# menyifang/MIMO

Measured on NVIDIA H100. Metric: frames/sec @ 512x512x24f, 20 DDIM steps, higher is better.
Workload: dtype fp16

## Files before the change

mimo_b200/csrc/gemm_wgmma.cu:

```cuda
#include <cuda_runtime.h>

#include <cudaTypedefs.h>

#include "../../include/mimo_b200.h"
#include "host_util.h"
#include "ptx.cuh"
#include "wgmma.cuh"

namespace mimo {

constexpr int BM = 128;
constexpr int BK = 64;
constexpr int kGemmThreads = 320;
constexpr int kChunk = 8192;

struct EpiArgs {
  const void* bias;
  const void* rowvec;
  long long rows_per_group;
  long long ld_rowvec;
  float scale;
  int act;
  float* partial;
};

struct ConvGeom {
  int conv;
  int H, W, NI;
  int TW, TH, TN;
  int tiles_w, tiles_h;
  int ctot;
  int c0;
  int kb0, kb1;
  int a_bytes;
  int chunk_bytes;
  int splits;
  int kb_split;
  int ntaps;
  signed char tdx[9], tdy[9];
};

template <int BN, bool kRes>
struct GemmCfg {
  static constexpr int kStageBytes = BM * BK * 2 + BN * BK * 2;
  static constexpr int kNChunk = BN / 32;
  static constexpr int kOutBytes = 2 * kChunk;
  static constexpr int kResSlots = kRes ? 2 : 0;
  static constexpr int kResBytes = kResSlots * kChunk;
  static constexpr int kBarBytes = 512;
  static constexpr int kFixed = kBarBytes + 2048  + kOutBytes + kResBytes;
  static constexpr int kMaxStages = (BN >= 256) ? 4 : (BN >= 160 ? 5 : (BN >= 128 ? 6 : 8));
  static constexpr int kFit = (227 * 1024 - kFixed) / kStageBytes;
  static constexpr int kStages = kFit < kMaxStages ? kFit : kMaxStages;
  static constexpr int kSmemBytes = kStages * kStageBytes + kFixed;
  static_assert(kStages >= 3, "pipeline too shallow");
};

template <int BN, bool kBf16, bool kRes>
__global__ void __launch_bounds__(kGemmThreads, 1)
gemm_wgmma_kernel(const __grid_constant__ CUtensorMap tmA0, const __grid_constant__ CUtensorMap tmA1,
                  const __grid_constant__ CUtensorMap tmB, const __grid_constant__ CUtensorMap tmOut,
                  const __grid_constant__ CUtensorMap tmRes, int M, int N, int num_m_tiles, int num_n_tiles,
                  int num_k_blocks, ConvGeom g, EpiArgs ep) {
  using Cfg = GemmCfg<BN, kRes>;
  using C = Cvt<kBf16>;
  using T = typename C::T;
  constexpr int NCHUNK = Cfg::kNChunk;
  extern __shared__ __align__(1024) uint8_t smem[];
  uint8_t* sOut = smem + Cfg::kStages * Cfg::kStageBytes;
  uint8_t* sRes = sOut + Cfg::kOutBytes;
  uint64_t* bars = reinterpret_cast<uint64_t*>(sRes + Cfg::kResBytes);
  uint64_t* full_bar = bars;
  uint64_t* empty_bar = bars + 8;
  uint64_t* res_full = bars + 16;
  uint64_t* res_empty = bars + 18;
  float* sbias = reinterpret_cast<float*>(reinterpret_cast<uint8_t*>(bars) + Cfg::kBarBytes);

  pdl_launch_dependents();
  const int warp = __shfl_sync(0xffffffffu, threadIdx.x >> 5, 0);
  const int lane = threadIdx.x & 31;
  const int num_tiles = num_m_tiles * num_n_tiles * g.splits;
  auto decode = [&](int tile, int& m_tile, int& n_tile, int& split, int& kb_begin, int& kb_cnt) {
    const int mn = tile / g.splits;
    split = tile - mn * g.splits;
    m_tile = mn / num_n_tiles;
    n_tile = mn - m_tile * num_n_tiles;
    kb_begin = split * g.kb_split;
    kb_cnt = num_k_blocks - kb_begin;
    if (kb_cnt > g.kb_split) kb_cnt = g.kb_split;
  };

  if (warp == 8 && lane == 0) {
    tma_prefetch_desc(&tmA0);
    tma_prefetch_desc(&tmA1);
    tma_prefetch_desc(&tmB);
    tma_prefetch_desc(&tmOut);
    if (kRes) tma_prefetch_desc(&tmRes);
  }
  if (warp == 9 && lane == 0) {
    for (int s = 0; s < Cfg::kStages; ++s) {
      mbar_init(&full_bar[s], 1);
      mbar_init(&empty_bar[s], 8);
    }
    for (int s = 0; s < Cfg::kResSlots; ++s) {
      mbar_init(&res_full[s], 1);
      mbar_init(&res_empty[s], 8);
    }
    fence_mbar_init();
  }
  __syncthreads();
  pdl_wait();

  auto tile_origin = [&](int m_tile, int& x0, int& y0, int& n0) {
    if (g.conv) {
      x0 = (m_tile % g.tiles_w) * g.TW;
      y0 = ((m_tile / g.tiles_w) % g.tiles_h) * g.TH;
      n0 = (m_tile / (g.tiles_w * g.tiles_h)) * g.TN;
    } else {
      x0 = y0 = n0 = 0;
    }
  };

  if (warp == 8) {
    uint32_t stage = 0, phase = 0;
    const int kb_per_tap = g.kb0 + g.kb1;
    for (int tile = blockIdx.x; tile < num_tiles; tile += gridDim.x) {
      int m_tile, n_tile, split, kb_begin, kb_cnt;
      decode(tile, m_tile, n_tile, split, kb_begin, kb_cnt);
      int x0, y0, n0;
      tile_origin(m_tile, x0, y0, n0);
      int tap = kb_per_tap > 0 ? kb_begin / kb_per_tap : 0;
      int rem = kb_begin - tap * kb_per_tap;
      int dx = g.tdx[tap], dy = g.tdy[tap], tap_k = tap * g.ctot;
      for (int kbl = 0, kb = kb_begin; kbl < kb_cnt; ++kbl, ++kb) {
        mbar_wait(&empty_bar[stage], phase ^ 1u);
        uint8_t* sa = smem + stage * Cfg::kStageBytes;
        uint8_t* sb = sa + BM * BK * 2;
        if (elect_one()) {
          if (!g.conv) {
            mbar_expect_tx(&full_bar[stage], BM * BK * 2 + BN * BK * 2);
            if (kb < g.kb0) {
              tma_load_2d(sa, &tmA0, &full_bar[stage], kb * BK, m_tile * BM);
              tma_load_2d(sb, &tmB, &full_bar[stage], kb * BK, n_tile * BN);
            } else {
              tma_load_2d(sa, &tmA1, &full_bar[stage], (kb - g.kb0) * BK, m_tile * BM);
              tma_load_2d(sb, &tmB, &full_bar[stage], g.c0 + (kb - g.kb0) * BK, n_tile * BN);
            }
          } else {
            mbar_expect_tx(&full_bar[stage], g.a_bytes + BN * BK * 2);
            int kcoord;
            if (rem < g.kb0) {
              tma_load_4d(sa, &tmA0, &full_bar[stage], rem * BK, x0 + dx, y0 + dy, n0);
              kcoord = tap_k + rem * BK;
            } else {
              tma_load_4d(sa, &tmA1, &full_bar[stage], (rem - g.kb0) * BK, x0 + dx, y0 + dy, n0);
              kcoord = tap_k + g.c0 + (rem - g.kb0) * BK;
            }
            tma_load_2d(sb, &tmB, &full_bar[stage], kcoord, n_tile * BN);
          }
        }
        __syncwarp();
        if (++rem == kb_per_tap) {
          rem = 0;
          tap_k += g.ctot;
          if (++tap == g.ntaps) tap = 0;
          dx = g.tdx[tap];
          dy = g.tdy[tap];
        }
        if (++stage == Cfg::kStages) {
          stage = 0;
          phase ^= 1u;
        }
      }
    }
  } else if (warp == 9) {
    if constexpr (kRes) {
      uint32_t k = 0;
      for (int tile = blockIdx.x; tile < num_tiles; tile += gridDim.x) {
        const int m_tile = tile / num_n_tiles;
        const int n_tile = tile % num_n_tiles;
        int x0, y0, n0;
        tile_origin(m_tile, x0, y0, n0);
        for (int c = 0; c < NCHUNK; ++c, ++k) {
          const uint32_t slot = k % Cfg::kResSlots;
          mbar_wait(&res_empty[slot], ((k / Cfg::kResSlots) & 1u) ^ 1u);
          if (elect_one()) {
            mbar_expect_tx(&res_full[slot], g.chunk_bytes);
            const int col = n_tile * BN + c * 32;
            if (g.conv)
              tma_load_4d(sRes + slot * kChunk, &tmRes, &res_full[slot], col, x0, y0, n0);
            else
              tma_load_2d(sRes + slot * kChunk, &tmRes, &res_full[slot], col, m_tile * BM);
          }
          __syncwarp();
        }
      }
    }
  } else if (warp < 8) {
    const int wg = warp >> 2;
    const int ct = threadIdx.x;
    const int rbase = wg * 64 + (warp & 3) * 16 + (lane >> 2);
    const int q2 = (lane & 3) * 2;
    const bool issuer = ct == 0;
    const int sw[2] = {(rbase >> 1) & 3, ((rbase + 8) >> 1) & 3};
    const bool do_silu = ep.act == MIMO_ACT_SILU;
    const uint32_t rpg = static_cast<uint32_t>(ep.rows_per_group);
    float acc[BN / 2];
    uint32_t stage = 0, phase = 0, lt = 0, oc = 0, rc = 0;

    for (int tile = blockIdx.x; tile < num_tiles; tile += gridDim.x, ++lt) {
      int m_tile, n_tile, split, kb_begin, kb_cnt;
      decode(tile, m_tile, n_tile, split, kb_begin, kb_cnt);
      int x0, y0, n0;
      tile_origin(m_tile, x0, y0, n0);
      auto tile_groups = [&](int mt, uint32_t& gf, uint32_t& gl) {
        if (!g.conv) {
          const uint32_t m0 = static_cast<uint32_t>(mt) * BM;
          uint32_t m1 = m0 + BM - 1;
          if (m1 > static_cast<uint32_t>(M) - 1) m1 = static_cast<uint32_t>(M) - 1;
          gf = m0 / rpg;
          gl = m1 / rpg;
        } else {
          int tx, ty, tn;
          tile_origin(mt, tx, ty, tn);
          int n1 = tn + g.TN - 1;
          if (n1 > g.NI - 1) n1 = g.NI - 1;
          const uint32_t hw = static_cast<uint32_t>(g.H) * g.W;
          gf = (static_cast<uint32_t>(tn) * hw) / rpg;
          gl = (static_cast<uint32_t>(n1 + 1) * hw - 1) / rpg;
        }
      };
      const int ce = ct;
      auto load_consts = [&](int t) -> float {
        float v = 0.f;
        const int mt = (t / g.splits) / num_n_tiles, nt = (t / g.splits) % num_n_tiles;
        const int col = nt * BN + ce;
        if (ce < BN && col < N) {
          if (ep.bias) v = C::to_f(static_cast<const T*>(ep.bias)[col]);
          if (ep.rowvec) {
            uint32_t gf, gl;
            tile_groups(mt, gf, gl);
            if (gf == gl) v += C::to_f(static_cast<const T*>(ep.rowvec)[static_cast<long long>(gf) * ep.ld_rowvec + col]);
          }
        }
        return ep.act == MIMO_ACT_GEGLU ? v : v * ep.scale;
      };
      float* sb = sbias + (lt & 1u) * 256;
      if (ct < BN) sb[ct] = load_consts(tile);

      uint32_t prev_stage = 0;
      for (int kb = 0; kb < kb_cnt; ++kb) {
        mbar_wait(&full_bar[stage], phase);
        const uint32_t sa = smem_u32(smem + stage * Cfg::kStageBytes);
        const uint64_t da = make_smem_desc_sw128(sa + wg * (64 * 128), 16, 1024);
        const uint64_t db = make_smem_desc_sw128(sa + BM * BK * 2, 16, 1024);
        wgmma_fence();
#pragma unroll
        for (int k = 0; k < BK / 16; ++k) {
          Wgmma<BN, kBf16>::ss(acc, da + 2 * k, db + 2 * k, (kb | k) != 0 ? 1u : 0u);
        }
        wgmma_commit();
        if (kb > 0) {
          wgmma_wait<1>();
          if (lane == 0) mbar_arrive(&empty_bar[prev_stage]);
        }
        prev_stage = stage;
        if (++stage == Cfg::kStages) {
          stage = 0;
          phase ^= 1u;
        }
      }
      wgmma_wait<0>();
      reg_fence(acc);
      if (lane == 0) mbar_arrive(&empty_bar[prev_stage]);

      long long row[2];
      bool row_ok[2];
#pragma unroll
      for (int h = 0; h < 2; ++h) {
        const int r = rbase + 8 * h;
        if (!g.conv) {
          row[h] = static_cast<long long>(m_tile) * BM + r;
          row_ok[h] = row[h] < M;
        } else {
          const int x = r % g.TW, y = (r / g.TW) % g.TH, n = r / (g.TW * g.TH);
          row_ok[h] = (n < g.TN) && (x0 + x < g.W) && (y0 + y < g.H) && (n0 + n < g.NI);
          row[h] = (static_cast<long long>(n0 + n) * g.H + (y0 + y)) * g.W + (x0 + x);
        }
      }
      asm volatile("bar.sync 1, 256;" ::: "memory");

      if (ep.partial) {
#pragma unroll
        for (int h = 0; h < 2; ++h) {
          if (!row_ok[h]) continue;
          float* prow = ep.partial + (static_cast<long long>(split) * M + row[h]) * N;
#pragma unroll
          for (int j = 0; j < BN / 8; ++j) {
            const int col = n_tile * BN + 8 * j + q2;
            if (col < N) *reinterpret_cast<float2*>(prow + col) = make_float2(acc[4 * j + 2 * h], acc[4 * j + 2 * h + 1]);
          }
        }
        continue;
      }

      auto stage_and_store = [&](uint8_t* obuf, int col0) {
        fence_proxy_async_smem();
        if (issuer) tma_store_wait_read0();
        asm volatile("bar.sync 1, 256;" ::: "memory");
        if (issuer) {
          if (g.conv)
            tma_store_4d(&tmOut, obuf, col0, x0, y0, n0);
          else
            tma_store_2d(&tmOut, obuf, col0, m_tile * BM);
          tma_store_commit();
        }
      };

      if (ep.act != MIMO_ACT_GEGLU) {
        const float scale = ep.scale;
        bool rv_uniform = false;
        if (ep.rowvec) {
          uint32_t gf, gl;
          tile_groups(m_tile, gf, gl);
          rv_uniform = gf == gl;
        }
        const bool need_rv = ep.rowvec != nullptr && !rv_uniform;
        const int mode = (!kRes && !do_silu && !need_rv && ep.bias == nullptr && ep.rowvec == nullptr && scale == 1.0f)
                             ? 0 : (need_rv ? 2 : 1);
        const T* rv[2];
#pragma unroll
        for (int h = 0; h < 2; ++h)
          rv[h] = (need_rv && row_ok[h])
                      ? static_cast<const T*>(ep.rowvec) + static_cast<long long>(static_cast<uint32_t>(row[h]) / rpg) * ep.ld_rowvec
                      : nullptr;
#pragma unroll
        for (int c = 0; c < NCHUNK; ++c) {
          uint8_t* obuf = sOut + (oc & 1u) * kChunk;
          ++oc;
          const int col0 = n_tile * BN + c * 32;
          [[maybe_unused]] uint32_t rslot = 0;
          if constexpr (kRes) {
            const uint32_t k = rc++;
            rslot = k % Cfg::kResSlots;
            mbar_wait(&res_full[rslot], (k / Cfg::kResSlots) & 1u);
          }
#pragma unroll
          for (int jj = 0; jj < 4; ++jj) {
            const int j = 4 * c + jj;
            const float2 cst0 = *reinterpret_cast<const float2*>(sb + c * 32 + 8 * jj + q2);
#pragma unroll
            for (int h = 0; h < 2; ++h) {
              const int r = rbase + 8 * h;
              const int off = r * 64 + ((jj ^ sw[h]) << 4) + q2 * 2;
              float f0 = acc[4 * j + 2 * h], f1 = acc[4 * j + 2 * h + 1];
              if (mode != 0) {
                float c0 = cst0.x, c1 = cst0.y;
                if (mode == 2 && rv[h] && col0 + 8 * jj + q2 < N) {
                  const float2 t = C::unpack(__ldg(reinterpret_cast<const unsigned int*>(rv[h] + col0 + 8 * jj + q2)));
                  c0 = fmaf(t.x, scale, c0);
                  c1 = fmaf(t.y, scale, c1);
                }
                f0 = fmaf(f0, scale, c0);
                f1 = fmaf(f1, scale, c1);
              }
              if constexpr (kRes) {
                const float2 t = C::unpack(*reinterpret_cast<const uint32_t*>(sRes + rslot * kChunk + off));
                f0 = fmaf(t.x, scale, f0);
                f1 = fmaf(t.y, scale, f1);
              }
              if (do_silu) {
                f0 = silu_f(f0);
                f1 = silu_f(f1);
              }
              *reinterpret_cast<uint32_t*>(obuf + off) = C::pack(f0, f1);
            }
          }
          if constexpr (kRes) {
            __syncwarp();
            if (lane == 0) mbar_arrive(&res_empty[rslot]);
          }
          stage_and_store(obuf, col0);
        }
      } else {
        constexpr int HALF = BN / 2;
#pragma unroll
        for (int c = 0; c < HALF / 32; ++c) {
          uint8_t* obuf = sOut + (oc & 1u) * kChunk;
          ++oc;
#pragma unroll
          for (int jj = 0; jj < 4; ++jj) {
            const int j = 4 * c + jj, jg = j + HALF / 8;
            const float2 cv = *reinterpret_cast<const float2*>(sb + c * 32 + 8 * jj + q2);
            const float2 cg = *reinterpret_cast<const float2*>(sb + HALF + c * 32 + 8 * jj + q2);
#pragma unroll
            for (int h = 0; h < 2; ++h) {
              const int r = rbase + 8 * h;
              const float f0 = (acc[4 * j + 2 * h] + cv.x) * gelu_erf_fast(acc[4 * jg + 2 * h] + cg.x);
              const float f1 = (acc[4 * j + 2 * h + 1] + cv.y) * gelu_erf_fast(acc[4 * jg + 2 * h + 1] + cg.y);
              *reinterpret_cast<uint32_t*>(obuf + r * 64 + ((jj ^ sw[h]) << 4) + q2 * 2) = C::pack(f0, f1);
            }
          }
          stage_and_store(obuf, n_tile * HALF + c * 32);
        }
      }
    }
    if (issuer) tma_store_wait_all();
  }
}


template <bool kBf16>
__global__ void __launch_bounds__(256)
splitk_reduce_kernel(const float* __restrict__ part, int splits, long long M, int N, const void* __restrict__ bias,
                     const void* __restrict__ rowvec, long long rpg, long long ld_rowvec,
                     const void* __restrict__ res, long long ld_res, float scale, int act, void* __restrict__ out,
                     long long ldo) {
  using C = Cvt<kBf16>;
  using T = typename C::T;
  pdl_launch_dependents();
  pdl_wait();
  const int nv = N >> 3;
  const long long idx = blockIdx.x * static_cast<long long>(blockDim.x) + threadIdx.x;
  if (idx >= M * nv) return;
  const long long row = idx / nv;
  const int col = static_cast<int>(idx - row * nv) * 8;
  float a[8] = {0.f, 0.f, 0.f, 0.f, 0.f, 0.f, 0.f, 0.f};
  for (int s = 0; s < splits; ++s) {
    const float4* p = reinterpret_cast<const float4*>(part + (static_cast<long long>(s) * M + row) * N + col);
    const float4 u0 = p[0], u1 = p[1];
    a[0] += u0.x, a[1] += u0.y, a[2] += u0.z, a[3] += u0.w;
    a[4] += u1.x, a[5] += u1.y, a[6] += u1.z, a[7] += u1.w;
  }
  float cst[8] = {0.f, 0.f, 0.f, 0.f, 0.f, 0.f, 0.f, 0.f};
  auto add_vec = [&](const T* v, float* dst, bool scaled_fma) {
    const uint4 b = *reinterpret_cast<const uint4*>(v);
    const uint32_t w[4] = {b.x, b.y, b.z, b.w};
#pragma unroll
    for (int j = 0; j < 4; ++j) {
      const float2 t = C::unpack(w[j]);
      if (scaled_fma) {
        dst[2 * j] = fmaf(t.x, scale, dst[2 * j]);
        dst[2 * j + 1] = fmaf(t.y, scale, dst[2 * j + 1]);
      } else {
        dst[2 * j] += t.x;
        dst[2 * j + 1] += t.y;
      }
    }
  };
  if (bias) add_vec(static_cast<const T*>(bias) + col, cst, false);
  if (rowvec) add_vec(static_cast<const T*>(rowvec) + (row / rpg) * ld_rowvec + col, cst, false);
  float f[8];
#pragma unroll
  for (int j = 0; j < 8; ++j) f[j] = fmaf(a[j], scale, cst[j] * scale);
  if (res) add_vec(static_cast<const T*>(res) + row * ld_res + col, f, true);
  if (act == MIMO_ACT_SILU) {
#pragma unroll
    for (int j = 0; j < 8; ++j) f[j] = silu_f(f[j]);
  }
  uint4 o;
  o.x = C::pack(f[0], f[1]);
  o.y = C::pack(f[2], f[3]);
  o.z = C::pack(f[4], f[5]);
  o.w = C::pack(f[6], f[7]);
  *reinterpret_cast<uint4*>(static_cast<T*>(out) + row * ldo + col) = o;
}

static int pick_splits(long long tiles, int nkb, long long M, int N, int64_t ws_bytes) {
  if (tiles * 2 > num_sms() || nkb < 32) return 1;
  long long s = num_sms() / tiles;
  if (s > nkb / 16) s = nkb / 16;
  if (s > 16) s = 16;
  while (s > 1 && s * M * N * 4 > ws_bytes) --s;
  return s < 2 ? 1 : static_cast<int>(s);
}

struct Maps {
  CUtensorMap a0, a1, b, out, res;
};

template <int BN, bool kBf16, bool kRes>
static int launch_cfg(const Maps& m, int M, int N, int mt, int nt, int nkb, const ConvGeom& g, const EpiArgs& ep,
                      cudaStream_t st) {
  using Cfg = GemmCfg<BN, kRes>;
  auto kern = gemm_wgmma_kernel<BN, kBf16, kRes>;
  static bool attr_done = false;
  if (!attr_done) {
    cudaError_t e = cudaFuncSetAttribute(kern, cudaFuncAttributeMaxDynamicSharedMemorySize, Cfg::kSmemBytes);
    if (e != cudaSuccess) return set_cuda_error("cudaFuncSetAttribute(gemm)", e);
    attr_done = true;
  }
  const int tiles = mt * nt;
  const int grid = tiles < num_sms() ? tiles : num_sms();
  cudaError_t e = launch_k(kern, dim3(grid), dim3(kGemmThreads), Cfg::kSmemBytes, st, m.a0, m.a1, m.b, m.out, m.res, M, N, mt,
                           nt, nkb, g, ep);
  if (e == cudaSuccess) e = cudaGetLastError();
  if (e != cudaSuccess) return set_cuda_error("gemm launch", e);
  return MIMO_OK;
}

template <bool kBf16>
static int launch_bn(int bn, bool res, const Maps& m, int M, int N, int mt, int nt, int nkb, const ConvGeom& g,
                     const EpiArgs& ep, cudaStream_t st) {
  switch (bn) {
    case 64:
      return res ? launch_cfg<64, kBf16, true>(m, M, N, mt, nt, nkb, g, ep, st)
                 : launch_cfg<64, kBf16, false>(m, M, N, mt, nt, nkb, g, ep, st);
    case 128:
      return res ? launch_cfg<128, kBf16, true>(m, M, N, mt, nt, nkb, g, ep, st)
                 : launch_cfg<128, kBf16, false>(m, M, N, mt, nt, nkb, g, ep, st);
    case 160:
      return res ? launch_cfg<160, kBf16, true>(m, M, N, mt, nt, nkb, g, ep, st)
                 : launch_cfg<160, kBf16, false>(m, M, N, mt, nt, nkb, g, ep, st);
    case 192:
      return res ? launch_cfg<192, kBf16, true>(m, M, N, mt, nt, nkb, g, ep, st)
                 : launch_cfg<192, kBf16, false>(m, M, N, mt, nt, nkb, g, ep, st);
    case 256:
      return res ? launch_cfg<256, kBf16, true>(m, M, N, mt, nt, nkb, g, ep, st)
                 : launch_cfg<256, kBf16, false>(m, M, N, mt, nt, nkb, g, ep, st);
  }
  return set_error(MIMO_ERR_ARG, "gemm: unsupported BN");
}

static int g_force_bn = 0;

int pick_bn(int N, bool geglu, long long m_tiles) {
  if (g_force_bn) return g_force_bn;
  if (geglu) {
    if (N % 256 == 0) return 256;
    if (N % 128 == 0) return 128;
    return 64;
  }
  const int cands[5] = {256, 192, 160, 128, 64};
  int best = 64;
  double best_eff = -1.0;
  for (int i = 0; i < 5; ++i) {
    const int bn = cands[i];
    const int nt = (N + bn - 1) / bn;
    double eff = static_cast<double>(N) / (static_cast<double>(nt) * bn);
    const long long tiles = m_tiles * nt;
    if (tiles < num_sms() && bn > 64) eff *= 0.5 + 0.5 * static_cast<double>(tiles) / num_sms();
    if (eff > best_eff + 1e-9) {
      best_eff = eff;
      best = bn;
    }
  }
  return best;
}

static EpiArgs make_epi(const mimo_epilogue& e, int N) {
  EpiArgs a;
  a.bias = e.bias;
  a.rowvec = e.rowvec;
  a.rows_per_group = e.rows_per_group > 0 ? e.rows_per_group : 1;
  if (a.rows_per_group > 0x7fffffffLL) a.rows_per_group = 0x7fffffffLL;
  a.ld_rowvec = e.ld_rowvec > 0 ? e.ld_rowvec : N;
  a.scale = e.scale;
  a.act = e.act;
  a.partial = nullptr;
  return a;
}

static int g_splitk = 0;

static int launch_reduce(int dtype, const float* part, int splits, long long M, int N, const mimo_epilogue& e, void* out,
                         long long ldo, cudaStream_t st) {
  const long long total = M * (N / 8);
  const unsigned blocks = div_up(total, 256);
  const long long rpg = e.rows_per_group > 0 ? e.rows_per_group : 1;
  const long long ldr = e.ld_rowvec > 0 ? e.ld_rowvec : N;
  cudaError_t err = dtype == MIMO_BF16
                        ? launch_k(splitk_reduce_kernel<true>, dim3(blocks), dim3(256), 0, st, part, splits, M, N, e.bias,
                                   e.rowvec, rpg, ldr, e.residual, static_cast<long long>(e.ld_res), e.scale, e.act, out, ldo)
                        : launch_k(splitk_reduce_kernel<false>, dim3(blocks), dim3(256), 0, st, part, splits, M, N, e.bias,
                                   e.rowvec, rpg, ldr, e.residual, static_cast<long long>(e.ld_res), e.scale, e.act, out, ldo);
  if (err == cudaSuccess) err = cudaGetLastError();
  if (err != cudaSuccess) return set_cuda_error("split-K reduce launch", err);
  return MIMO_OK;
}

}

using namespace mimo;

extern "C" int mimo_debug_splitk(int mode) {
  g_splitk = mode;
  return 0;
}

extern "C" int mimo_debug_force_bn(int bn) {
  g_force_bn = bn;
  return 0;
}

extern "C" int mimo_gemm_geglu_granule(int32_t N) { return pick_bn(N, true, 1 << 20) / 2; }

extern "C" int mimo_gemm(const mimo_gemm_params* p, void* stream) {
  if (!p || !p->a || !p->w || !p->out) return set_error(MIMO_ERR_ARG, "mimo_gemm: null pointer");
  if (p->M <= 0 || p->N <= 0 || p->K <= 0) return set_error(MIMO_ERR_ARG, "mimo_gemm: empty problem");
  if ((p->K % 8) || (p->lda % 8) || (p->ldw % 8) || (p->N % 8) || (p->ldo % 8))
    return set_error(MIMO_ERR_ARG, "mimo_gemm: K, N, lda, ldw, ldo must be multiples of 8");
  if (p->ep.residual && (p->ep.ld_res % 8)) return set_error(MIMO_ERR_ARG, "mimo_gemm: ld_res % 8 != 0");
  const bool geglu = p->ep.act == MIMO_ACT_GEGLU;
  if (geglu && (p->ep.residual || p->ep.rowvec))
    return set_error(MIMO_ERR_ARG, "mimo_gemm: GEGLU takes neither a residual nor a row vector");
  if (int rc = ensure_device()) return rc;
  const int mt = (p->M + BM - 1) / BM;
  const int K1 = p->a1 ? p->K1 : 0;
  if (K1 < 0 || (K1 % 8) || (p->a1 && (p->lda1 % 8))) return set_error(MIMO_ERR_ARG, "mimo_gemm: K1/lda1 % 8 != 0");
  const int kb0 = (p->K + BK - 1) / BK;
  const int kb1 = (K1 + BK - 1) / BK;
  const int nkb = kb0 + kb1;
  int bn = pick_bn(p->N, geglu, mt);
  int splits = 1;
  if (!geglu && g_splitk && p->workspace && !g_force_bn) {
    const int bn_wide = pick_bn(p->N, false, 1 << 20);
    splits = pick_splits(static_cast<long long>(mt) * ((p->N + bn_wide - 1) / bn_wide), nkb, p->M, p->N, p->workspace_bytes);
    if (splits > 1) bn = bn_wide;
  }
  if (geglu && (p->N % bn)) return set_error(MIMO_ERR_ARG, "mimo_gemm: GEGLU needs N % tile == 0");
  const int nt = (p->N + bn - 1) / bn;
  const bool res = p->ep.residual != nullptr && !geglu && splits == 1;

  Maps m;
  const uint64_t adim[2] = {static_cast<uint64_t>(p->K), static_cast<uint64_t>(p->M)};
  const uint64_t astr[1] = {static_cast<uint64_t>(p->lda) * 2};
  const uint32_t abox[2] = {BK, BM};
  if (int rc = encode_tmap(&m.a0, p->dtype, 2, p->a, adim, astr, abox)) return rc;
  m.a1 = m.a0;
  if (K1) {
    const uint64_t a1dim[2] = {static_cast<uint64_t>(K1), static_cast<uint64_t>(p->M)};
    const uint64_t a1str[1] = {static_cast<uint64_t>(p->lda1) * 2};
    if (int rc = encode_tmap(&m.a1, p->dtype, 2, p->a1, a1dim, a1str, abox)) return rc;
  }
  const uint64_t bdim[2] = {static_cast<uint64_t>(p->K + K1), static_cast<uint64_t>(p->N)};
  const uint64_t bstr[1] = {static_cast<uint64_t>(p->ldw) * 2};
  const uint32_t bbox[2] = {BK, static_cast<uint32_t>(bn)};
  if (int rc = encode_tmap(&m.b, p->dtype, 2, p->w, bdim, bstr, bbox)) return rc;
  const int n_out = geglu ? p->N / 2 : p->N;
  const uint64_t odim[2] = {static_cast<uint64_t>(n_out), static_cast<uint64_t>(p->M)};
  const uint64_t ostr[1] = {static_cast<uint64_t>(p->ldo) * 2};
  const uint32_t obox[2] = {32, BM};
  if (int rc = encode_tmap(&m.out, p->dtype, 2, p->out, odim, ostr, obox, 64)) return rc;
  m.res = m.out;
  if (res) {
    const uint64_t rstr[1] = {static_cast<uint64_t>(p->ep.ld_res) * 2};
    if (int rc = encode_tmap(&m.res, p->dtype, 2, p->ep.residual, odim, rstr, obox, 64)) return rc;
  }

  ConvGeom g = {};
  g.kb0 = kb0;
  g.kb1 = kb1;
  g.c0 = p->K;
  g.chunk_bytes = kChunk;
  g.splits = splits;
  g.kb_split = (nkb + splits - 1) / splits;
  EpiArgs ep = make_epi(p->ep, p->N);
  cudaStream_t st = static_cast<cudaStream_t>(stream);
  if (splits > 1) {
    ep.bias = ep.rowvec = nullptr;
    ep.act = MIMO_ACT_NONE;
    ep.scale = 1.0f;
    ep.partial = static_cast<float*>(p->workspace);
  }
  const int rc = p->dtype == MIMO_BF16 ? launch_bn<true>(bn, res, m, p->M, p->N, mt, nt, nkb, g, ep, st)
                                       : launch_bn<false>(bn, res, m, p->M, p->N, mt, nt, nkb, g, ep, st);
  if (rc || splits == 1) return rc;
  return launch_reduce(p->dtype, ep.partial, splits, p->M, p->N, p->ep, p->out, p->ldo, st);
}

static int conv_launch(const mimo_conv3x3_params* p, const void* w, int ntaps, const signed char* tdx,
                       const signed char* tdy, void* out, int sx, int sy, int ow, int oh, void* stream) {
  const int c1 = p->x1 ? p->c1 : 0;
  ConvGeom g = {};
  g.conv = 1;
  g.H = p->h;
  g.W = p->w_;
  g.NI = p->n;
  g.TW = p->w_ < BM ? p->w_ : BM;
  g.TH = BM / g.TW;
  if (g.TH > p->h) g.TH = p->h;
  if (g.TH < 1) g.TH = 1;
  g.TN = BM / (g.TW * g.TH);
  if (g.TN > p->n) g.TN = p->n;
  if (g.TN < 1) g.TN = 1;
  if (g.TN > 1 && g.TH != p->h) g.TN = 1;
  g.tiles_w = (p->w_ + g.TW - 1) / g.TW;
  g.tiles_h = (p->h + g.TH - 1) / g.TH;
  const int tiles_n = (p->n + g.TN - 1) / g.TN;
  g.ctot = p->c0 + c1;
  g.c0 = p->c0;
  g.kb0 = (p->c0 + BK - 1) / BK;
  g.kb1 = (c1 + BK - 1) / BK;
  g.a_bytes = g.TW * g.TH * g.TN * BK * 2;
  g.chunk_bytes = g.TW * g.TH * g.TN * 64;
  g.ntaps = ntaps;
  for (int t = 0; t < 9; ++t) {
    g.tdx[t] = t < ntaps ? tdx[t] : 0;
    g.tdy[t] = t < ntaps ? tdy[t] : 0;
  }
  const int mt = g.tiles_w * g.tiles_h * tiles_n;
  const int nkb = ntaps * (g.kb0 + g.kb1);
  const long long Mrows = static_cast<long long>(p->n) * p->h * p->w_;
  if (Mrows > 0x7fffffffLL) return set_error(MIMO_ERR_ARG, "mimo_conv: too many pixels");
  int bn = pick_bn(p->cout, false, mt);
  int splits = 1;
  if (g_splitk && p->workspace && !g_force_bn && sx == 1 && sy == 1 && p->ldo == p->cout) {
    const int bn_wide = pick_bn(p->cout, false, 1 << 20);
    splits = pick_splits(static_cast<long long>(mt) * ((p->cout + bn_wide - 1) / bn_wide), nkb, Mrows, p->cout,
// ... 87 lines not shown
```

mimo_b200/csrc/ptx.cuh:

```cuda
#pragma once
#include <cuda_fp16.h>
#include <cuda_bf16.h>
#include <cuda.h>
#include <stdint.h>
#include <stdio.h>

namespace mimo {

__device__ __forceinline__ uint32_t smem_u32(const void* p) {
  return static_cast<uint32_t>(__cvta_generic_to_shared(p));
}
__device__ __forceinline__ uint32_t lane_id() { return threadIdx.x & 31u; }

__device__ __forceinline__ bool elect_one() {
  uint32_t pred = 0;
  asm volatile(
      "{\n\t.reg .pred P;\n\telect.sync _|P, 0xffffffff;\n\tselp.u32 %0, 1, 0, P;\n\t}\n"
      : "=r"(pred));
  return pred != 0;
}

__device__ __forceinline__ void pdl_launch_dependents() { asm volatile("griddepcontrol.launch_dependents;" ::: "memory"); }
__device__ __forceinline__ void pdl_wait() { asm volatile("griddepcontrol.wait;" ::: "memory"); }

__device__ __forceinline__ void mbar_init(uint64_t* bar, uint32_t count) {
  asm volatile("mbarrier.init.shared::cta.b64 [%0], %1;" ::"r"(smem_u32(bar)), "r"(count));
}
__device__ __forceinline__ void fence_mbar_init() {
  asm volatile("fence.mbarrier_init.release.cluster;" ::: "memory");
}
__device__ __forceinline__ void mbar_expect_tx(uint64_t* bar, uint32_t bytes) {
  asm volatile("mbarrier.arrive.expect_tx.shared::cta.b64 _, [%0], %1;" ::"r"(smem_u32(bar)),
               "r"(bytes)
               : "memory");
}
__device__ __forceinline__ void mbar_arrive(uint64_t* bar) {
  asm volatile("mbarrier.arrive.shared::cta.b64 _, [%0];" ::"r"(smem_u32(bar)) : "memory");
}
__device__ __forceinline__ bool mbar_try_wait(uint64_t* bar, uint32_t parity) {
  uint32_t ok;
  asm volatile(
      "{\n\t.reg .pred p;\n\t"
      "mbarrier.try_wait.parity.shared::cta.b64 p, [%1], %2;\n\t"
      "selp.u32 %0, 1, 0, p;\n\t}\n"
      : "=r"(ok)
      : "r"(smem_u32(bar)), "r"(parity)
      : "memory");
  return ok != 0;
}
__device__ __forceinline__ bool mbar_test(uint64_t* bar, uint32_t parity) {
  uint32_t ok;
  asm volatile(
      "{\n\t.reg .pred p;\n\t"
      "mbarrier.test_wait.parity.shared::cta.b64 p, [%1], %2;\n\t"
      "selp.u32 %0, 1, 0, p;\n\t}\n"
      : "=r"(ok)
      : "r"(smem_u32(bar)), "r"(parity)
      : "memory");
  return ok != 0;
}
__device__ __forceinline__ void mbar_wait(uint64_t* bar, uint32_t parity) {
  uint32_t spins = 0;
  while (!mbar_try_wait(bar, parity)) {
    if (++spins > (1u << 26)) __trap();
  }
}

__device__ __forceinline__ void fence_proxy_async_smem() {
  asm volatile("fence.proxy.async.shared::cta;" ::: "memory");
}

__device__ __forceinline__ void tma_prefetch_desc(const CUtensorMap* m) {
  asm volatile("prefetch.tensormap [%0];" ::"l"(reinterpret_cast<uint64_t>(m)) : "memory");
}
__device__ __forceinline__ void tma_load_2d(void* smem_dst, const CUtensorMap* m, uint64_t* bar,
                                            int32_t c0, int32_t c1) {
  asm volatile(
      "cp.async.bulk.tensor.2d.shared::cluster.global.mbarrier::complete_tx::bytes"
      " [%0], [%1, {%3, %4}], [%2];"
      ::"r"(smem_u32(smem_dst)), "l"(reinterpret_cast<uint64_t>(m)), "r"(smem_u32(bar)), "r"(c0),
      "r"(c1)
      : "memory");
}
__device__ __forceinline__ void tma_load_3d(void* smem_dst, const CUtensorMap* m, uint64_t* bar,
                                            int32_t c0, int32_t c1, int32_t c2) {
  asm volatile(
      "cp.async.bulk.tensor.3d.shared::cluster.global.mbarrier::complete_tx::bytes"
      " [%0], [%1, {%3, %4, %5}], [%2];"
      ::"r"(smem_u32(smem_dst)), "l"(reinterpret_cast<uint64_t>(m)), "r"(smem_u32(bar)), "r"(c0),
      "r"(c1), "r"(c2)
      : "memory");
}
__device__ __forceinline__ void tma_load_4d(void* smem_dst, const CUtensorMap* m, uint64_t* bar,
                                            int32_t c0, int32_t c1, int32_t c2, int32_t c3) {
  asm volatile(
      "cp.async.bulk.tensor.4d.shared::cluster.global.mbarrier::complete_tx::bytes"
      " [%0], [%1, {%3, %4, %5, %6}], [%2];"
      ::"r"(smem_u32(smem_dst)), "l"(reinterpret_cast<uint64_t>(m)), "r"(smem_u32(bar)), "r"(c0),
      "r"(c1), "r"(c2), "r"(c3)
      : "memory");
}

__device__ __forceinline__ void tma_store_2d(const CUtensorMap* m, const void* smem_src, int32_t c0, int32_t c1) {
  asm volatile("cp.async.bulk.tensor.2d.global.shared::cta.bulk_group [%0, {%2, %3}], [%1];"
               ::"l"(reinterpret_cast<uint64_t>(m)), "r"(smem_u32(smem_src)), "r"(c0), "r"(c1)
               : "memory");
}
__device__ __forceinline__ void tma_store_4d(const CUtensorMap* m, const void* smem_src, int32_t c0, int32_t c1,
                                             int32_t c2, int32_t c3) {
  asm volatile("cp.async.bulk.tensor.4d.global.shared::cta.bulk_group [%0, {%2, %3, %4, %5}], [%1];"
               ::"l"(reinterpret_cast<uint64_t>(m)), "r"(smem_u32(smem_src)), "r"(c0), "r"(c1), "r"(c2), "r"(c3)
               : "memory");
}
__device__ __forceinline__ void tma_store_commit() { asm volatile("cp.async.bulk.commit_group;" ::: "memory"); }
__device__ __forceinline__ void tma_store_wait_read0() { asm volatile("cp.async.bulk.wait_group.read 0;" ::: "memory"); }
__device__ __forceinline__ void tma_store_wait_all() { asm volatile("cp.async.bulk.wait_group 0;" ::: "memory"); }

__device__ __forceinline__ void wgmma_fence() { asm volatile("wgmma.fence.sync.aligned;" ::: "memory"); }
__device__ __forceinline__ void wgmma_commit() { asm volatile("wgmma.commit_group.sync.aligned;" ::: "memory"); }
template <int N>
__device__ __forceinline__ void wgmma_wait() {
  asm volatile("wgmma.wait_group.sync.aligned %0;" ::"n"(N) : "memory");
}
template <int N>
__device__ __forceinline__ void reg_fence(float (&d)[N]) {
#pragma unroll
  for (int i = 0; i < N; ++i) asm volatile("" : "+f"(d[i])::"memory");
}

__device__ __forceinline__ void bar_sync(int id, int count) {
  asm volatile("bar.sync %0, %1;" ::"r"(id), "r"(count) : "memory");
}
__device__ __forceinline__ void bar_arrive(int id, int count) {
  asm volatile("bar.arrive %0, %1;" ::"r"(id), "r"(count) : "memory");
}

__device__ __forceinline__ uint64_t make_smem_desc_sw128(uint32_t smem_addr, uint32_t lbo_bytes,
                                                         uint32_t sbo_bytes) {
  uint64_t d = 0;
  d |= static_cast<uint64_t>((smem_addr & 0x3FFFFu) >> 4);
  d |= static_cast<uint64_t>((lbo_bytes >> 4) & 0x3FFFu) << 16;
  d |= static_cast<uint64_t>((sbo_bytes >> 4) & 0x3FFFu) << 32;
  d |= static_cast<uint64_t>(1) << 62;
  return d;
}

__device__ __forceinline__ float ex2_ftz(float x) {
  float y;
  asm("ex2.approx.ftz.f32 %0, %1;" : "=f"(y) : "f"(x));
  return y;
}
__device__ __forceinline__ float silu_f(float x) { return __fdividef(x, 1.0f + __expf(-x)); }
__device__ __forceinline__ float gelu_erf_f(float x) {
  return 0.5f * x * (1.0f + erff(x * 0.70710678118654752440f));
}

__device__ __forceinline__ float gelu_erf_fast(float x) {
  const float z = fabsf(x) * 0.70710678118654752440f;
  float t;
  asm("rcp.approx.ftz.f32 %0, %1;" : "=f"(t) : "f"(fmaf(0.3275911f, z, 1.0f)));
  float poly = fmaf(1.061405429f, t, -1.453152027f);
  poly = fmaf(poly, t, 1.421413741f);
  poly = fmaf(poly, t, -0.284496736f);
  poly = fmaf(poly, t, 0.254829592f);
  poly *= t;
  float e;
  asm("ex2.approx.ftz.f32 %0, %1;" : "=f"(e) : "f"(-z * z * 1.4426950408889634f));
  const float erf_abs = fmaf(-poly, e, 1.0f);
  const float erf_v = copysignf(erf_abs, x);
  return 0.5f * x * (1.0f + erf_v);
}

template <bool kBf16>
struct Cvt;
template <>
struct Cvt<false> {
  using T = __half;
  using T2 = __half2;
  static __device__ __forceinline__ float to_f(T v) { return __half2float(v); }
  static __device__ __forceinline__ T from_f(float v) { return __float2half_rn(v); }
  static __device__ __forceinline__ uint32_t pack(float a, float b) {
    __half2 h = __floats2half2_rn(a, b);
    return *reinterpret_cast<uint32_t*>(&h);
  }
  static __device__ __forceinline__ float2 unpack(uint32_t u) {
    return __half22float2(*reinterpret_cast<__half2*>(&u));
  }
};
template <>
struct Cvt<true> {
  using T = __nv_bfloat16;
  using T2 = __nv_bfloat162;
  static __device__ __forceinline__ float to_f(T v) { return __bfloat162float(v); }
  static __device__ __forceinline__ T from_f(float v) { return __float2bfloat16_rn(v); }
  static __device__ __forceinline__ uint32_t pack(float a, float b) {
    __nv_bfloat162 h = __floats2bfloat162_rn(a, b);
    return *reinterpret_cast<uint32_t*>(&h);
  }
  static __device__ __forceinline__ float2 unpack(uint32_t u) {
    return __bfloat1622float2(*reinterpret_cast<__nv_bfloat162*>(&u));
  }
};

}
```

Before: 8.128.

## Add ping-pong consumer warpgroups with register reallocation to WGMMA GEMM

For narrower tiles, the two consumer warpgroups now each own a whole 128-row tile (two 64-row wgmma halves) and alternate tiles, so one group's epilogue overlaps the other's main loop, ordered through named barriers. The block grows to 384 threads, and setmaxnreg moves registers from the producer warps to the consumers. The output staging, residual rings and bias buffers are duplicated per owner, and a done barrier keeps producers alive until consumers finish. The costs are a doubled accumulator footprint, more shared memory for the fixed buffers (possibly fewer pipeline stages), and more complex synchronisation.

```diff
diff --git a/mimo_b200/csrc/gemm_wgmma.cu b/mimo_b200/csrc/gemm_wgmma.cu
--- a/mimo_b200/csrc/gemm_wgmma.cu
+++ b/mimo_b200/csrc/gemm_wgmma.cu
@@ -11,7 +11,9 @@
 
 constexpr int BM = 128;
 constexpr int BK = 64;
-constexpr int kGemmThreads = 320;
+constexpr int kGemmThreads = 384;
+constexpr int kConsumerRegs = 232;
+constexpr int kProducerRegs = 40;
 constexpr int kChunk = 8192;
 
 struct EpiArgs {
@@ -42,13 +44,17 @@
 
 template <int BN, bool kRes>
 struct GemmCfg {
+  static constexpr bool kPingPong = BN < 192 || (BN == 192 && !kRes);
+  static constexpr int kMH = kPingPong ? 2 : 1;
+  static constexpr int kOwners = kPingPong ? 2 : 1;
   static constexpr int kStageBytes = BM * BK * 2 + BN * BK * 2;
   static constexpr int kNChunk = BN / 32;
-  static constexpr int kOutBytes = 2 * kChunk;
+  static constexpr int kOutBytes = kOwners * 2 * kChunk;
   static constexpr int kResSlots = kRes ? 2 : 0;
-  static constexpr int kResBytes = kResSlots * kChunk;
+  static constexpr int kResBytes = kOwners * kResSlots * kChunk;
   static constexpr int kBarBytes = 512;
-  static constexpr int kFixed = kBarBytes + 2048  + kOutBytes + kResBytes;
+  static constexpr int kConstBytes = kOwners * 2 * 256 * 4;
+  static constexpr int kFixed = kBarBytes + kConstBytes + kOutBytes + kResBytes;
   static constexpr int kMaxStages = (BN >= 256) ? 4 : (BN >= 160 ? 5 : (BN >= 128 ? 6 : 8));
   static constexpr int kFit = (227 * 1024 - kFixed) / kStageBytes;
   static constexpr int kStages = kFit < kMaxStages ? kFit : kMaxStages;
@@ -66,6 +72,9 @@
   using C = Cvt<kBf16>;
   using T = typename C::T;
   constexpr int NCHUNK = Cfg::kNChunk;
+  constexpr bool kPP = Cfg::kPingPong;
+  constexpr int MH = Cfg::kMH;
+  constexpr int kConsumerWarps = kPP ? 4 : 8;
   extern __shared__ __align__(1024) uint8_t smem[];
   uint8_t* sOut = smem + Cfg::kStages * Cfg::kStageBytes;
   uint8_t* sRes = sOut + Cfg::kOutBytes;
@@ -73,7 +82,8 @@
   uint64_t* full_bar = bars;
   uint64_t* empty_bar = bars + 8;
   uint64_t* res_full = bars + 16;
-  uint64_t* res_empty = bars + 18;
+  uint64_t* res_empty = bars + 20;
+  uint64_t* done_bar = bars + 24;
   float* sbias = reinterpret_cast<float*>(reinterpret_cast<uint8_t*>(bars) + Cfg::kBarBytes);
 
   pdl_launch_dependents();
@@ -100,12 +110,13 @@
   if (warp == 9 && lane == 0) {
     for (int s = 0; s < Cfg::kStages; ++s) {
       mbar_init(&full_bar[s], 1);
-      mbar_init(&empty_bar[s], 8);
+      mbar_init(&empty_bar[s], kConsumerWarps);
     }
-    for (int s = 0; s < Cfg::kResSlots; ++s) {
+    for (int s = 0; s < Cfg::kOwners * Cfg::kResSlots; ++s) {
       mbar_init(&res_full[s], 1);
-      mbar_init(&res_empty[s], 8);
+      mbar_init(&res_empty[s], kConsumerWarps);
     }
+    mbar_init(done_bar, 8);
     fence_mbar_init();
   }
   __syncthreads();
@@ -121,96 +132,121 @@
     }
   };
 
-  if (warp == 8) {
-    uint32_t stage = 0, phase = 0;
-    const int kb_per_tap = g.kb0 + g.kb1;
-    for (int tile = blockIdx.x; tile < num_tiles; tile += gridDim.x) {
-      int m_tile, n_tile, split, kb_begin, kb_cnt;
-      decode(tile, m_tile, n_tile, split, kb_begin, kb_cnt);
-      int x0, y0, n0;
-      tile_origin(m_tile, x0, y0, n0);
-      int tap = kb_per_tap > 0 ? kb_begin / kb_per_tap : 0;
-      int rem = kb_begin - tap * kb_per_tap;
-      int dx = g.tdx[tap], dy = g.tdy[tap], tap_k = tap * g.ctot;
-      for (int kbl = 0, kb = kb_begin; kbl < kb_cnt; ++kbl, ++kb) {
-        mbar_wait(&empty_bar[stage], phase ^ 1u);
-        uint8_t* sa = smem + stage * Cfg::kStageBytes;
-        uint8_t* sb = sa + BM * BK * 2;
-        if (elect_one()) {
-          if (!g.conv) {
-            mbar_expect_tx(&full_bar[stage], BM * BK * 2 + BN * BK * 2);
-            if (kb < g.kb0) {
-              tma_load_2d(sa, &tmA0, &full_bar[stage], kb * BK, m_tile * BM);
-              tma_load_2d(sb, &tmB, &full_bar[stage], kb * BK, n_tile * BN);
+  if (warp >= 8) {
+    setmaxnreg_dec<kProducerRegs>();
+    if (warp == 8) {
+      uint32_t stage = 0, phase = 0;
+      const int kb_per_tap = g.kb0 + g.kb1;
+      for (int tile = blockIdx.x; tile < num_tiles; tile += gridDim.x) {
+        int m_tile, n_tile, split, kb_begin, kb_cnt;
+        decode(tile, m_tile, n_tile, split, kb_begin, kb_cnt);
+        int x0, y0, n0;
+        tile_origin(m_tile, x0, y0, n0);
+        int tap = kb_per_tap > 0 ? kb_begin / kb_per_tap : 0;
+        int rem = kb_begin - tap * kb_per_tap;
+        int dx = g.tdx[tap], dy = g.tdy[tap], tap_k = tap * g.ctot;
+        for (int kbl = 0, kb = kb_begin; kbl < kb_cnt; ++kbl, ++kb) {
+          mbar_wait(&empty_bar[stage], phase ^ 1u);
+          uint8_t* sa = smem + stage * Cfg::kStageBytes;
+          uint8_t* sb = sa + BM * BK * 2;
+          if (elect_one()) {
+            if (!g.conv) {
+              mbar_expect_tx(&full_bar[stage], BM * BK * 2 + BN * BK * 2);
+              if (kb < g.kb0) {
+                tma_load_2d(sa, &tmA0, &full_bar[stage], kb * BK, m_tile * BM);
+                tma_load_2d(sb, &tmB, &full_bar[stage], kb * BK, n_tile * BN);
+              } else {
+                tma_load_2d(sa, &tmA1, &full_bar[stage], (kb - g.kb0) * BK, m_tile * BM);
+                tma_load_2d(sb, &tmB, &full_bar[stage], g.c0 + (kb - g.kb0) * BK, n_tile * BN);
+              }
             } else {
-              tma_load_2d(sa, &tmA1, &full_bar[stage], (kb - g.kb0) * BK, m_tile * BM);
-              tma_load_2d(sb, &tmB, &full_bar[stage], g.c0 + (kb - g.kb0) * BK, n_tile * BN);
+              mbar_expect_tx(&full_bar[stage], g.a_bytes + BN * BK * 2);
+              int kcoord;
+              if (rem < g.kb0) {
+                tma_load_4d(sa, &tmA0, &full_bar[stage], rem * BK, x0 + dx, y0 + dy, n0);
+                kcoord = tap_k + rem * BK;
+              } else {
+                tma_load_4d(sa, &tmA1, &full_bar[stage], (rem - g.kb0) * BK, x0 + dx, y0 + dy, n0);
+                kcoord = tap_k + g.c0 + (rem - g.kb0) * BK;
+              }
+              tma_load_2d(sb, &tmB, &full_bar[stage], kcoord, n_tile * BN);
             }
-          } else {
-            mbar_expect_tx(&full_bar[stage], g.a_bytes + BN * BK * 2);
-            int kcoord;
-            if (rem < g.kb0) {
-              tma_load_4d(sa, &tmA0, &full_bar[stage], rem * BK, x0 + dx, y0 + dy, n0);
-              kcoord = tap_k + rem * BK;
-            } else {
-              tma_load_4d(sa, &tmA1, &full_bar[stage], (rem - g.kb0) * BK, x0 + dx, y0 + dy, n0);
-              kcoord = tap_k + g.c0 + (rem - g.kb0) * BK;
+          }
+          __syncwarp();
+          if (++rem == kb_per_tap) {
+            rem = 0;
+            tap_k += g.ctot;
+            if (++tap == g.ntaps) tap = 0;
+            dx = g.tdx[tap];
+            dy = g.tdy[tap];
+          }
+          if (++stage == Cfg::kStages) {
+            stage = 0;
+            phase ^= 1u;
+          }
+        }
+      }
+      mbar_wait(done_bar, 0);
+    } else if (warp >= 9 && warp - 9 < Cfg::kOwners) {
+      if constexpr (kRes) {
+        const uint32_t own = warp - 9;
+        uint8_t* ring = sRes + own * (Cfg::kResSlots * kChunk);
+        uint64_t* rfull = res_full + own * Cfg::kResSlots;
+        uint64_t* rempty = res_empty + own * Cfg::kResSlots;
+        uint32_t k = 0, lt = 0;
+        for (int tile = blockIdx.x; tile < num_tiles; tile += gridDim.x, ++lt) {
+          if (kPP && (lt & 1u) != own) continue;
+          const int m_tile = tile / num_n_tiles;
+          const int n_tile = tile % num_n_tiles;
+          int x0, y0, n0;
+          tile_origin(m_tile, x0, y0, n0);
+          for (int c = 0; c < NCHUNK; ++c, ++k) {
+            const uint32_t slot = k % Cfg::kResSlots;
+            mbar_wait(&rempty[slot], ((k / Cfg::kResSlots) & 1u) ^ 1u);
+            if (elect_one()) {
+              mbar_expect_tx(&rfull[slot], g.chunk_bytes);
+              const int col = n_tile * BN + c * 32;
+              if (g.conv)
+                tma_load_4d(ring + slot * kChunk, &tmRes, &rfull[slot], col, x0, y0, n0);
+              else
+                tma_load_2d(ring + slot * kChunk, &tmRes, &rfull[slot], col, m_tile * BM);
             }
-            tma_load_2d(sb, &tmB, &full_bar[stage], kcoord, n_tile * BN);
-          }
-        }
-        __syncwarp();
-        if (++rem == kb_per_tap) {
-          rem = 0;
-          tap_k += g.ctot;
-          if (++tap == g.ntaps) tap = 0;
-          dx = g.tdx[tap];
-          dy = g.tdy[tap];
-        }
-        if (++stage == Cfg::kStages) {
-          stage = 0;
-          phase ^= 1u;
+            __syncwarp();
+          }
         }
       }
     }
-  } else if (warp == 9) {
-    if constexpr (kRes) {
-      uint32_t k = 0;
-      for (int tile = blockIdx.x; tile < num_tiles; tile += gridDim.x) {
-        const int m_tile = tile / num_n_tiles;
-        const int n_tile = tile % num_n_tiles;
-        int x0, y0, n0;
-        tile_origin(m_tile, x0, y0, n0);
-        for (int c = 0; c < NCHUNK; ++c, ++k) {
-          const uint32_t slot = k % Cfg::kResSlots;
-          mbar_wait(&res_empty[slot], ((k / Cfg::kResSlots) & 1u) ^ 1u);
-          if (elect_one()) {
-            mbar_expect_tx(&res_full[slot], g.chunk_bytes);
-            const int col = n_tile * BN + c * 32;
-            if (g.conv)
-              tma_load_4d(sRes + slot * kChunk, &tmRes, &res_full[slot], col, x0, y0, n0);
-            else
-              tma_load_2d(sRes + slot * kChunk, &tmRes, &res_full[slot], col, m_tile * BM);
-          }
-          __syncwarp();
-        }
-      }
-    }
-  } else if (warp < 8) {
+  } else {
+    setmaxnreg_inc<kConsumerRegs>();
     const int wg = warp >> 2;
     const int ct = threadIdx.x;
-    const int rbase = wg * 64 + (warp & 3) * 16 + (lane >> 2);
+    const int wt = kPP ? (ct & 127) : ct;
+    constexpr int kTileThreads = kPP ? 128 : 256;
+    const int own = kPP ? wg : 0;
+    const int epi_bar = kPP ? 4 + wg : 1;
+    const int rbase = (kPP ? 0 : wg * 64) + (warp & 3) * 16 + (lane >> 2);
     const int q2 = (lane & 3) * 2;
-    const bool issuer = ct == 0;
-    const int sw[2] = {(rbase >> 1) & 3, ((rbase + 8) >> 1) & 3};
+    const bool issuer = wt == 0;
+    const int sw = (rbase >> 1) & 3;
     const bool do_silu = ep.act == MIMO_ACT_SILU;
     const uint32_t rpg = static_cast<uint32_t>(ep.rows_per_group);
-    float acc[BN / 2];
-    uint32_t stage = 0, phase = 0, lt = 0, oc = 0, rc = 0;
+    uint8_t* sOutOwn = sOut + own * (2 * kChunk);
+    uint8_t* ring = sRes + own * (Cfg::kResSlots * kChunk);
+    uint64_t* rfull = res_full + own * Cfg::kResSlots;
+    uint64_t* rempty = res_empty + own * Cfg::kResSlots;
+    float acc[MH][BN / 2];
+    uint32_t stage = 0, phase = 0, lt = 0, ot = 0, oc = 0, rc = 0;
+    if (kPP && wg == 1) bar_arrive(2, 256);
 
     for (int tile = blockIdx.x; tile < num_tiles; tile += gridDim.x, ++lt) {
       int m_tile, n_tile, split, kb_begin, kb_cnt;
       decode(tile, m_tile, n_tile, split, kb_begin, kb_cnt);
+      if (kPP && (lt & 1u) != static_cast<uint32_t>(wg)) {
+        stage += kb_cnt;
+        phase ^= (stage / Cfg::kStages) & 1u;
+        stage %= Cfg::kStages;
+        continue;
+      }
       int x0, y0, n0;
       tile_origin(m_tile, x0, y0, n0);
       auto tile_groups = [&](int mt, uint32_t& gf, uint32_t& gl) {
@@ -230,8 +266,7 @@
           gl = (static_cast<uint32_t>(n1 + 1) * hw - 1) / rpg;
         }
       };
-      const int ce = ct;
-      auto load_consts = [&](int t) -> float {
+      auto load_consts = [&](int t, int ce) -> float {
         float v = 0.f;
         const int mt = (t / g.splits) / num_n_tiles, nt = (t / g.splits) % num_n_tiles;
         const int col = nt * BN + ce;
@@ -245,19 +280,24 @@
         }
         return ep.act == MIMO_ACT_GEGLU ? v : v * ep.scale;
       };
-      float* sb = sbias + (lt & 1u) * 256;
-      if (ct < BN) sb[ct] = load_consts(tile);
-
+      float* sb = sbias + (own * 2 + (ot & 1u)) * 256;
+      ++ot;
+      for (int ce = wt; ce < BN; ce += kTileThreads) sb[ce] = load_consts(tile, ce);
+
+      if (kPP) bar_sync(2 + wg, 256);
       uint32_t prev_stage = 0;
       for (int kb = 0; kb < kb_cnt; ++kb) {
-        mbar_wait(&full_bar[stage], phase);
+        mbar_wait_spin(&full_bar[stage], phase);
         const uint32_t sa = smem_u32(smem + stage * Cfg::kStageBytes);
-        const uint64_t da = make_smem_desc_sw128(sa + wg * (64 * 128), 16, 1024);
         const uint64_t db = make_smem_desc_sw128(sa + BM * BK * 2, 16, 1024);
         wgmma_fence();
 #pragma unroll
         for (int k = 0; k < BK / 16; ++k) {
-          Wgmma<BN, kBf16>::ss(acc, da + 2 * k, db + 2 * k, (kb | k) != 0 ? 1u : 0u);
+#pragma unroll
+          for (int mh = 0; mh < MH; ++mh) {
+            const uint64_t da = make_smem_desc_sw128(sa + (kPP ? mh : wg) * (64 * 128), 16, 1024);
+            Wgmma<BN, kBf16>::ss(acc[mh], da + 2 * k, db + 2 * k, (kb | k) != 0 ? 1u : 0u);
+          }
         }
         wgmma_commit();
         if (kb > 0) {
@@ -270,44 +310,51 @@
           phase ^= 1u;
         }
       }
+      if (kPP && tile + static_cast<int>(gridDim.x) < num_tiles) bar_arrive(3 - wg, 256);
       wgmma_wait<0>();
-      reg_fence(acc);
+#pragma unroll
+      for (int mh = 0; mh < MH; ++mh) reg_fence(acc[mh]);
       if (lane == 0) mbar_arrive(&empty_bar[prev_stage]);
 
-      long long row[2];
-      bool row_ok[2];
-#pragma unroll
-      for (int h = 0; h < 2; ++h) {
-        const int r = rbase + 8 * h;
-        if (!g.conv) {
-          row[h] = static_cast<long long>(m_tile) * BM + r;
-          row_ok[h] = row[h] < M;
-        } else {
-          const int x = r % g.TW, y = (r / g.TW) % g.TH, n = r / (g.TW * g.TH);
-          row_ok[h] = (n < g.TN) && (x0 + x < g.W) && (y0 + y < g.H) && (n0 + n < g.NI);
-          row[h] = (static_cast<long long>(n0 + n) * g.H + (y0 + y)) * g.W + (x0 + x);
-        }
-      }
-      asm volatile("bar.sync 1, 256;" ::: "memory");
+      long long row[MH][2];
+      bool row_ok[MH][2];
+#pragma unroll
+      for (int mh = 0; mh < MH; ++mh)
+#pragma unroll
+        for (int h = 0; h < 2; ++h) {
+          const int r = rbase + 64 * mh + 8 * h;
+          if (!g.conv) {
+            row[mh][h] = static_cast<long long>(m_tile) * BM + r;
+            row_ok[mh][h] = row[mh][h] < M;
+          } else {
+            const int x = r % g.TW, y = (r / g.TW) % g.TH, n = r / (g.TW * g.TH);
+            row_ok[mh][h] = (n < g.TN) && (x0 + x < g.W) && (y0 + y < g.H) && (n0 + n < g.NI);
+            row[mh][h] = (static_cast<long long>(n0 + n) * g.H + (y0 + y)) * g.W + (x0 + x);
+          }
+        }
+      bar_sync(epi_bar, kTileThreads);
 
       if (ep.partial) {
 #pragma unroll
-        for (int h = 0; h < 2; ++h) {
-          if (!row_ok[h]) continue;
-          float* prow = ep.partial + (static_cast<long long>(split) * M + row[h]) * N;
-#pragma unroll
-          for (int j = 0; j < BN / 8; ++j) {
-            const int col = n_tile * BN + 8 * j + q2;
-            if (col < N) *reinterpret_cast<float2*>(prow + col) = make_float2(acc[4 * j + 2 * h], acc[4 * j + 2 * h + 1]);
-          }
-        }
+        for (int mh = 0; mh < MH; ++mh)
+#pragma unroll
+          for (int h = 0; h < 2; ++h) {
+            if (!row_ok[mh][h]) continue;
+            float* prow = ep.partial + (static_cast<long long>(split) * M + row[mh][h]) * N;
+#pragma unroll
+            for (int j = 0; j < BN / 8; ++j) {
+              const int col = n_tile * BN + 8 * j + q2;
+              if (col < N)
+                *reinterpret_cast<float2*>(prow + col) = make_float2(acc[mh][4 * j + 2 * h], acc[mh][4 * j + 2 * h + 1]);
+            }
+          }
         continue;
       }
 
       auto stage_and_store = [&](uint8_t* obuf, int col0) {
         fence_proxy_async_smem();
         if (issuer) tma_store_wait_read0();
-        asm volatile("bar.sync 1, 256;" ::: "memory");
+        bar_sync(epi_bar, kTileThreads);
         if (issuer) {
           if (g.conv)
             tma_store_4d(&tmOut, obuf, col0, x0, y0, n0);
@@ -328,57 +375,63 @@
         const bool need_rv = ep.rowvec != nullptr && !rv_uniform;
         const int mode = (!kRes && !do_silu && !need_rv && ep.bias == nullptr && ep.rowvec == nullptr && scale == 1.0f)
                              ? 0 : (need_rv ? 2 : 1);
-        const T* rv[2];
-#pragma unroll
-        for (int h = 0; h < 2; ++h)
-          rv[h] = (need_rv && row_ok[h])
-                      ? static_cast<const T*>(ep.rowvec) + static_cast<long long>(static_cast<uint32_t>(row[h]) / rpg) * ep.ld_rowvec
-                      : nullptr;
+        const T* rv[MH][2];
+#pragma unroll
+        for (int mh = 0; mh < MH; ++mh)
+#pragma unroll
+          for (int h = 0; h < 2; ++h)
+            rv[mh][h] = (need_rv && row_ok[mh][h])
+                            ? static_cast<const T*>(ep.rowvec) +
+                                  static_cast<long long>(static_cast<uint32_t>(row[mh][h]) / rpg) * ep.ld_rowvec
+                            : nullptr;
 #pragma unroll
         for (int c = 0; c < NCHUNK; ++c) {
-          uint8_t* obuf = sOut + (oc & 1u) * kChunk;
+          uint8_t* obuf = sOutOwn + (oc & 1u) * kChunk;
           ++oc;
           const int col0 = n_tile * BN + c * 32;
           [[maybe_unused]] uint32_t rslot = 0;
           if constexpr (kRes) {
             const uint32_t k = rc++;
             rslot = k % Cfg::kResSlots;
-            mbar_wait(&res_full[rslot], (k / Cfg::kResSlots) & 1u);
+            mbar_wait_spin(&rfull[rslot], (k / Cfg::kResSlots) & 1u);
           }
 #pragma unroll
           for (int jj = 0; jj < 4; ++jj) {
             const int j = 4 * c + jj;
             const float2 cst0 = *reinterpret_cast<const float2*>(sb + c * 32 + 8 * jj + q2);
 #pragma unroll
-            for (int h = 0; h < 2; ++h) {
-              const int r = rbase + 8 * h;
-              const int off = r * 64 + ((jj ^ sw[h]) << 4) + q2 * 2;
-              float f0 = acc[4 * j + 2 * h], f1 = acc[4 * j + 2 * h + 1];
-              if (mode != 0) {
-                float c0 = cst0.x, c1 = cst0.y;
-                if (mode == 2 && rv[h] && col0 + 8 * jj + q2 < N) {
-                  const float2 t = C::unpack(__ldg(reinterpret_cast<const unsigned int*>(rv[h] + col0 + 8 * jj + q2)));
-                  c0 = fmaf(t.x, scale, c0);
-                  c1 = fmaf(t.y, scale, c1);
+            for (int mh = 0; mh < MH; ++mh)
+#pragma unroll
+              for (int h = 0; h < 2; ++h) {
+                const int r = rbase + 64 * mh + 8 * h;
+                const int off = r * 64 + ((jj ^ sw) << 4) + q2 * 2;
+                float f0 = acc[mh][4 * j + 2 * h], f1 = acc[mh][4 * j + 2 * h + 1];
+                if (mode != 0) {
+                  float c0 = cst0.x, c1 = cst0.y;
+                  if (mode == 2 && rv[mh][h] && col0 + 8 * jj + q2 < N) {
+                    const float2 t =
+                        C::unpack(__ldg(reinterpret_cast<const unsigned int*>(rv[mh][h] + col0 + 8 * jj + q2)));
+                    c0 = fmaf(t.x, scale, c0);
+                    c1 = fmaf(t.y, scale, c1);
+                  }
+                  f0 = fmaf(f0, scale, c0);
+                  f1 = fmaf(f1, scale, c1);
                 }
-                f0 = fmaf(f0, scale, c0);
-                f1 = fmaf(f1, scale, c1);
+                if constexpr (kRes) {
+                  const float2 t = C::unpack(*reinterpret_cast<const uint32_t*>(ring + rslot * kChunk + off));
+                  f0 = fmaf(t.x, scale, f0);
+                  f1 = fmaf(t.y, scale, f1);
+                }
+                if (do_silu) {
+                  f0 = silu_f(f0);
+                  f1 = silu_f(f1);
+                }
+                *reinterpret_cast<uint32_t*>(obuf + off) = C::pack(f0, f1);
               }
-              if constexpr (kRes) {
-                const float2 t = C::unpack(*reinterpret_cast<const uint32_t*>(sRes + rslot * kChunk + off));
-                f0 = fmaf(t.x, scale, f0);
-                f1 = fmaf(t.y, scale, f1);
-              }
-              if (do_silu) {
-                f0 = silu_f(f0);
-                f1 = silu_f(f1);
-              }
-              *reinterpret_cast<uint32_t*>(obuf + off) = C::pack(f0, f1);
-            }
           }
           if constexpr (kRes) {
             __syncwarp();
-            if (lane == 0) mbar_arrive(&res_empty[rslot]);
+            if (lane == 0) mbar_arrive(&rempty[rslot]);
           }
           stage_and_store(obuf, col0);
         }
@@ -386,7 +439,7 @@
         constexpr int HALF = BN / 2;
 #pragma unroll
         for (int c = 0; c < HALF / 32; ++c) {
-          uint8_t* obuf = sOut + (oc & 1u) * kChunk;
+          uint8_t* obuf = sOutOwn + (oc & 1u) * kChunk;
           ++oc;
 #pragma unroll
           for (int jj = 0; jj < 4; ++jj) {
@@ -394,17 +447,21 @@
             const float2 cv = *reinterpret_cast<const float2*>(sb + c * 32 + 8 * jj + q2);
             const float2 cg = *reinterpret_cast<const float2*>(sb + HALF + c * 32 + 8 * jj + q2);
 #pragma unroll
-            for (int h = 0; h < 2; ++h) {
-              const int r = rbase + 8 * h;
-              const float f0 = (acc[4 * j + 2 * h] + cv.x) * gelu_erf_fast(acc[4 * jg + 2 * h] + cg.x);
-              const float f1 = (acc[4 * j + 2 * h + 1] + cv.y) * gelu_erf_fast(acc[4 * jg + 2 * h + 1] + cg.y);
-              *reinterpret_cast<uint32_t*>(obuf + r * 64 + ((jj ^ sw[h]) << 4) + q2 * 2) = C::pack(f0, f1);
-            }
+            for (int mh = 0; mh < MH; ++mh)
+#pragma unroll
+              for (int h = 0; h < 2; ++h) {
+                const int r = rbase + 64 * mh + 8 * h;
+                const float f0 = (acc[mh][4 * j + 2 * h] + cv.x) * gelu_erf_fast(acc[mh][4 * jg + 2 * h] + cg.x);
+                const float f1 =
+                    (acc[mh][4 * j + 2 * h + 1] + cv.y) * gelu_erf_fast(acc[mh][4 * jg + 2 * h + 1] + cg.y);
+                *reinterpret_cast<uint32_t*>(obuf + r * 64 + ((jj ^ sw) << 4) + q2 * 2) = C::pack(f0, f1);
+              }
           }
           stage_and_store(obuf, n_tile * HALF + c * 32);
         }
       }
     }
+    if (lane == 0) mbar_arrive(done_bar);
     if (issuer) tma_store_wait_all();
   }
 }
diff --git a/mimo_b200/csrc/ptx.cuh b/mimo_b200/csrc/ptx.cuh
--- a/mimo_b200/csrc/ptx.cuh
+++ b/mimo_b200/csrc/ptx.cuh
@@ -65,6 +65,10 @@
     if (++spins > (1u << 26)) __trap();
   }
 }
+__device__ __forceinline__ void mbar_wait_spin(uint64_t* bar, uint32_t parity) {
+  while (!mbar_try_wait(bar, parity)) {
+  }
+}
 
 __device__ __forceinline__ void fence_proxy_async_smem() {
   asm volatile("fence.proxy.async.shared::cta;" ::: "memory");
@@ -126,6 +130,15 @@
 __device__ __forceinline__ void reg_fence(float (&d)[N]) {
 #pragma unroll
   for (int i = 0; i < N; ++i) asm volatile("" : "+f"(d[i])::"memory");
+}
+
+template <int N>
+__device__ __forceinline__ void setmaxnreg_inc() {
+  asm volatile("setmaxnreg.inc.sync.aligned.u32 %0;" ::"n"(N));
+}
+template <int N>
+__device__ __forceinline__ void setmaxnreg_dec() {
+  asm volatile("setmaxnreg.dec.sync.aligned.u32 %0;" ::"n"(N));
 }
 
 __device__ __forceinline__ void bar_sync(int id, int count) {
```

Result: no change. 8.152, median of 6 (+0.3%).
